# ElusAegis/metal-msm-gpu-acceleration

Hardware: AMD Instinct MI355X
Metric: BN254 G1 MSM/s at log_size=20 (5 instances) (higher is better)
Workload: dtype u32x8 (256-bit Montgomery integer)

## Files before the change

metal-msm-gpu-acceleration_amd/csrc/bn254_fq29.hip.h:

```cpp
#pragma once
#include "bn254_fq.hip.h"

namespace msm_amd {

struct fe29 {
  uint32_t l[9];
};

MSM_HD uint32_t limb32(uint32_t x) {
#if defined(__HIP_DEVICE_COMPILE__) && !defined(MSM_FQ29_NOPIN)
  asm("" : "+v"(x));
#endif
  return x;
}
MSM_HD fe29 pin_limbs(const fe29& a) {
  fe29 r;
#if defined(__HIP_DEVICE_COMPILE__)
  _Pragma("unroll") for (int i = 0; i < 9; ++i) r.l[i] = limb32(a.l[i]);
#else
  r = a;
#endif
  return r;
}

#if defined(__HIP_DEVICE_COMPILE__)
#define MSM_ISA_MARK(name) asm volatile("; MSM_MARK " name)
#else
#define MSM_ISA_MARK(name) ((void)0)
#endif

enum KSel { K4E30 = 0, K8E30 = 1, K8E31 = 2, K16E30 = 3, K16E31 = 4, K12E30 = 5 };

struct Fq29 {
  static constexpr uint32_t MASK = 0x1FFFFFFFu;
  static constexpr uint32_t INV = 0x04866389u;
  static constexpr uint32_t PINV = 0x1B799C77u;

  MSM_HD static constexpr uint32_t p(int i) {
    constexpr uint32_t c[9] = {0x187CFD47u, 0x010460B6u, 0x1C72A34Fu, 0x02D522D0u, 0x1585D978u,
                               0x02DB40C0u, 0x00A6E141u, 0x0E5C2634u, 0x0030644Eu};
    return c[i];
  }
  MSM_HD static constexpr uint32_t one_c(int i) {
    constexpr uint32_t c[9] = {0x157CCC21u, 0x141C2758u, 0x185230D3u, 0x014C0419u, 0x0AA36FB9u,
                               0x1D4240CEu, 0x11D54C07u, 0x052AC7A8u, 0x000DC836u};
    return c[i];
  }
  MSM_HD static constexpr uint32_t cin_c(int i) {
    constexpr uint32_t c[9] = {0x13349CA1u, 0x1A5D84A8u, 0x0A3E5CACu, 0x100249E0u, 0x12B951E8u,
                               0x0E92D304u, 0x14CB95B3u, 0x041B9D3Du, 0x00058003u};
    return c[i];
  }
  MSM_HD static constexpr uint32_t dout_c(int i) {
    constexpr uint32_t c[9] = {0x058F0D9Du, 0x1AEA1C6Eu, 0x11C2CF74u, 0x11D651EBu, 0x1462C0A7u,
                               0x11B7BC3Cu, 0x1CBD99BAu, 0x183340FBu, 0x000E0A77u};
    return c[i];
  }
  MSM_HD static constexpr uint32_t kc(int sel, int i) {
    constexpr uint32_t c[6][9] = {
        {0x41F3F51Cu, 0x441182D9u, 0x51CA8D3Au, 0x4B548B41u, 0x561765DEu, 0x4B6D0300u, 0x429B8502u, 0x597098CEu, 0x00C19137u},
        {0x43E7EA38u, 0x482305B4u, 0x43951A76u, 0x56A91685u, 0x4C2ECBBEu, 0x56DA0603u, 0x45370A06u, 0x52E1319Eu, 0x01832271u},
        {0x83E7EA38u, 0x882305B2u, 0x83951A74u, 0x96A91683u, 0x8C2ECBBCu, 0x96DA0601u, 0x85370A04u, 0x92E1319Cu, 0x0183226Fu},
        {0x47CFD470u, 0x50460B6Au, 0x472A34EEu, 0x4D522D0Cu, 0x585D977Fu, 0x4DB40C08u, 0x4A6E140Fu, 0x45C2633Eu, 0x030644E5u},
        {0x87CFD470u, 0x90460B68u, 0x872A34ECu, 0x8D522D0Au, 0x985D977Du, 0x8DB40C06u, 0x8A6E140Du, 0x85C2633Cu, 0x030644E3u},
        {0x45DBDF54u, 0x4C34888Fu, 0x555FA7B2u, 0x41FDA1C8u, 0x4246319Fu, 0x42470906u, 0x47D28F0Bu, 0x4C51CA6Eu, 0x0244B3ABu}};
    return c[sel][i];
  }

  MSM_HD static fe29 zero() {
    fe29 r;
    MSM_UNROLL for (int i = 0; i < 9; ++i) r.l[i] = 0;
    return r;
  }
  MSM_HD static fe29 one() {
    fe29 r;
    MSM_UNROLL for (int i = 0; i < 9; ++i) r.l[i] = one_c(i);
    return r;
  }
  MSM_HD static bool is_zero_limbs(const fe29& a) {
    uint32_t o = 0;
    MSM_UNROLL for (int i = 0; i < 9; ++i) o |= a.l[i];
    return o == 0;
  }

  MSM_HD static fe29 add(const fe29& a, const fe29& b) {
    fe29 r;
    MSM_UNROLL for (int i = 0; i < 9; ++i) r.l[i] = a.l[i] + b.l[i];
    return r;
  }

  template <int SEL>
  MSM_HD static fe29 sub(const fe29& a, const fe29& b) {
    fe29 r;
    MSM_UNROLL for (int i = 0; i < 9; ++i) r.l[i] = (a.l[i] + kc(SEL, i)) - b.l[i];
    return r;
  }

  MSM_HD static fe29 neg(const fe29& a) { return norm(sub<K4E30>(zero(), a)); }
  MSM_HD static fe29 neg_wide(const fe29& a) { return sub<K4E30>(zero(), a); }

  MSM_HD static fe29 norm(const fe29& a) {
    fe29 r;
    r.l[0] = a.l[0] & MASK;
    MSM_UNROLL for (int i = 1; i < 8; ++i) r.l[i] = (a.l[i] & MASK) + (a.l[i - 1] >> 29);
    r.l[8] = a.l[8] + (a.l[7] >> 29);
    return r;
  }

  template <bool WIDE = false>
  MSM_HD static fe29 reduce_columns(uint64_t (&A)[17]) {
    uint64_t carry = 0;
    MSM_UNROLL for (int k = 0; k < 9; ++k) {
      A[k] += carry;
      const uint32_t m = (WIDE && k < 8) ? (uint32_t)A[k] * INV : ((uint32_t)A[k] * INV) & MASK;
      MSM_UNROLL for (int j = 0; j < 9; ++j) A[k + j] += (uint64_t)m * p(j);
      carry = A[k] >> 29;
    }
    fe29 r;
    MSM_UNROLL for (int k = 9; k < 17; ++k) {
      A[k] += carry;
      r.l[k - 9] = (uint32_t)A[k] & MASK;
      carry = A[k] >> 29;
    }
    r.l[8] = (uint32_t)carry;
    return r;
  }


#if defined(MSM_AMD_EXPERIMENTS)
#include "experiments/fq29_variants.inc"
#endif

  template <bool PIN = true, bool WIDE = false>
  MSM_HD static fe29 mul(const fe29& a_in, const fe29& b_in) {
    const fe29 a = PIN ? pin_limbs(a_in) : a_in, b = PIN ? pin_limbs(b_in) : b_in;
#if defined(MSM_AMD_EXPERIMENTS) && defined(MSM_FQ29_FIPS)
    {
      const fe29* const xs[1] = {&a};
      const fe29* const ys[1] = {&b};
      return fips<1>(xs, ys);
    }
#endif
    uint64_t A[17];
    MSM_UNROLL for (int k = 0; k < 17; ++k) {
      uint64_t s = 0;
      MSM_UNROLL for (int i = 0; i < 9; ++i) {
        const int j = k - i;
        if (j >= 0 && j < 9) s += (uint64_t)a.l[i] * b.l[j];
      }
      A[k] = s;
    }
    return reduce_columns<WIDE>(A);
  }

  template <bool PIN = true, bool WIDE = false>
  MSM_HD static fe29 mul2(const fe29& a_in, const fe29& b_in, const fe29& c_in, const fe29& d_in) {
    const fe29 a = PIN ? pin_limbs(a_in) : a_in, b = PIN ? pin_limbs(b_in) : b_in, c = PIN ? pin_limbs(c_in) : c_in,
               d = PIN ? pin_limbs(d_in) : d_in;
#if defined(MSM_AMD_EXPERIMENTS) && defined(MSM_FQ29_FIPS)
    {
      const fe29* const xs[2] = {&a, &c};
      const fe29* const ys[2] = {&b, &d};
      return fips<2>(xs, ys);
    }
#endif
    uint64_t A[17];
    MSM_UNROLL for (int k = 0; k < 17; ++k) {
      uint64_t s = 0;
      MSM_UNROLL for (int i = 0; i < 9; ++i) {
        const int j = k - i;
        if (j >= 0 && j < 9) {
          s += (uint64_t)a.l[i] * b.l[j];
          s += (uint64_t)c.l[i] * d.l[j];
        }
      }
      A[k] = s;
    }
    return reduce_columns<WIDE>(A);
  }

  template <bool PIN = true, bool WIDE = false>
  MSM_HD static fe29 sqr(const fe29& a_in) {
    const fe29 a = PIN ? pin_limbs(a_in) : a_in;
#if defined(MSM_AMD_EXPERIMENTS) && defined(MSM_FQ29_FIPS)
    {
      fe29 d2;
      MSM_UNROLL for (int i = 0; i < 9; ++i) d2.l[i] = a.l[i] << 1;
      const fe29* const xs[1] = {&d2};
      const fe29* const ys[1] = {&a};
      return fips<1, true>(xs, ys);
    }
#endif
    uint32_t d[9];
    MSM_UNROLL for (int i = 0; i < 9; ++i) d[i] = a.l[i] << 1;
    uint64_t A[17];
    MSM_UNROLL for (int k = 0; k < 17; ++k) {
      uint64_t s = 0;
      MSM_UNROLL for (int i = 0; i < 9; ++i) {
        const int j = k - i;
        if (j >= 0 && j < 9 && i < j) s += (uint64_t)d[i] * a.l[j];
      }
      if ((k & 1) == 0) s += (uint64_t)a.l[k >> 1] * a.l[k >> 1];
      A[k] = s;
    }
    return reduce_columns<WIDE>(A);
  }
  MSM_HD static fe29 mul_np(const fe29& a, const fe29& b) { return mul<false, true>(a, b); }
  MSM_HD static fe29 sqr_np(const fe29& a) { return sqr<false, true>(a); }
  MSM_HD static fe29 mul2_np(const fe29& a, const fe29& b, const fe29& c, const fe29& d) { return mul2<false>(a, b, c, d); }
  MSM_HD static fe29 mul2w_np(const fe29& a, const fe29& b, const fe29& c, const fe29& d) {
    return mul2<false, true>(a, b, c, d);
  }

  MSM_HD static fe29 unpack256(const u256& x) {
    fe29 t;
    MSM_UNROLL for (int i = 0; i < 9; ++i) {
      const int bit = 29 * i;
      const int w = bit >> 5, s = bit & 31;
      uint32_t v = x.v[w] >> s;
      if (s > 3 && w + 1 < 8) v |= x.v[w + 1] << (32 - s);
      t.l[i] = (i < 8) ? (v & MASK) : v;
    }
    return t;
  }

  template <int SH>
  MSM_HD static fe29 unpack256_shl(const u256& x) {
    static_assert(SH >= 0 && SH <= 3, "the top limb holds 232 - SH .. 255 of x");
    fe29 t;
    t.l[0] = (x.v[0] << SH) & MASK;
    MSM_UNROLL for (int i = 1; i < 9; ++i) {
      const int bit = 29 * i - SH;
      const int w = bit >> 5, s = bit & 31;
      uint32_t v = x.v[w] >> s;
      if (s > 3 && w + 1 < 8) v |= x.v[w + 1] << (32 - s);
      t.l[i] = (i < 8) ? (v & MASK) : v;
    }
    return t;
  }

  MSM_HD static u256 pack256(const fe29& t) {
    u256 r;
    MSM_UNROLL for (int w = 0; w < 8; ++w) {
      const int bit = 32 * w;
      const int i = bit / 29, s = bit % 29;
      uint32_t v = t.l[i] >> s;
      if (i + 1 < 9) v |= t.l[i + 1] << (29 - s);
      if (29 - s + 29 < 32 && i + 2 < 9) v |= t.l[i + 2] << (58 - s);
      r.v[w] = v;
    }
    return r;
  }

  MSM_HD static fe29 from_ext(const u256& x) {
    fe29 c;
    MSM_UNROLL for (int i = 0; i < 9; ++i) c.l[i] = cin_c(i);
    return mul(unpack256(x), c);
  }

  MSM_HD static fe29 canonical(const fe29& a, int rounds) {
    fe29 r;
    uint32_t carry = 0;
    MSM_UNROLL for (int i = 0; i < 8; ++i) {
      const uint64_t s = (uint64_t)a.l[i] + carry;
      r.l[i] = (uint32_t)s & MASK;
      carry = (uint32_t)(s >> 29);
    }
    r.l[8] = a.l[8] + carry;
    for (int it = 0; it < rounds; ++it) {
      fe29 d;
      int32_t borrow = 0;
      MSM_UNROLL for (int i = 0; i < 9; ++i) {
        const int32_t s = (int32_t)r.l[i] - (int32_t)p(i) + borrow;
        d.l[i] = (i < 8) ? ((uint32_t)s & MASK) : (uint32_t)s;
        borrow = (i < 8) ? (s >> 29) : 0;
        if (i == 8) borrow = (s < 0) ? -1 : 0;
      }
      if (borrow == 0) r = d;
    }
    return r;
  }

  MSM_HD static u256 to_ext(const fe29& a) {
    fe29 d;
    MSM_UNROLL for (int i = 0; i < 9; ++i) d.l[i] = dout_c(i);
    return pack256(canonical(mul(a, d), 1));
  }

  MSM_HD static u256 pack_canonical(const fe29& a) { return pack256(canonical(a, 1)); }

  MSM_HD static bool maybe_zero(const fe29& a, uint32_t bound) {
    return (((a.l[0] & MASK) * PINV) & MASK) < bound;
  }

  MSM_HD static bool is_zero_exact(const fe29& a) {
    const fe29 t = canonical(mul(a, one()), 1);
    return is_zero_limbs(t);
  }
};

}
```

metal-msm-gpu-acceleration_amd/csrc/k_accumulate.hip:

```cpp
#include "device_common.hip.h"
#include "launch.h"
#include "point_stages.hip.h"

namespace msm_amd {

struct PackedBases {
  using Rec = AffPacked;
  static constexpr bool kIso = false;
  static __device__ __forceinline__ bool is_identity(const Rec& r) { return affpacked_is_identity(r); }
  static __device__ __forceinline__ AffI unpack(const Rec& r) { return affi_unpack_finite(r); }
  static __device__ __forceinline__ fe29 neg_y(const fe29& y) { return Fq29::neg_wide(y); }
};
struct ExtBases {
  using Rec = Affine;
  static constexpr bool kIso = true;
  static __device__ __forceinline__ bool is_identity(const Rec& r) { return affine_words_zero(r); }
  static __device__ __forceinline__ AffI unpack(const Rec& r) { return affi_from_ext_iso(r); }
  static __device__ __forceinline__ fe29 neg_y(const fe29& y) { return neg_wide_iso(y); }
};
template <bool PIN, class B>
__device__ __forceinline__ void
accumulate_item(const uint32_t slot, const typename B::Rec* __restrict__ bases, const uint32_t* __restrict__ sorted,
                   const uint32_t* __restrict__ bucket_start, const uint32_t* __restrict__ bucket_size,
                   const uint32_t* __restrict__ item_start, const uint32_t* __restrict__ win_base,
                   const uint2* __restrict__ order, const PlanCounters* __restrict__ counters, uint32_t n,
                   uint32_t lb, uint32_t CH, PtI* __restrict__ buckets, PtI* __restrict__ partials) {
  if (PIN) asm volatile("v_mov_b32 v175, 0" ::: "v175");
  if (slot >= counters->total_items) return;
  const uint2 it = order[slot];
  const uint32_t b = it.x, j = it.y;
  const uint32_t w = b >> lb;
  const uint32_t size = bucket_size[b];
  const uint32_t lo = j * CH;
  const uint32_t cnt = min(size - lo, CH);
  const uint32_t* idx = sorted + (size_t)w * n + bucket_start[b] + lo;
  PtI acc = pti_identity();
  enum : uint32_t { kEmpty = 0, kOne = 1, kMany = 2 };
  uint32_t state = kEmpty;
  uint32_t cur_idx = idx[0];
  uint32_t next_idx = cnt > 1 ? idx[1] : 0u;
  using Rec = typename B::Rec;
  Rec pre;
  pre.x = load_u256(&bases[cur_idx & 0x7FFFFFFFu].x);
  pre.y = load_u256(&bases[cur_idx & 0x7FFFFFFFu].y);
  uint32_t i = 0;
  auto signed_point = [](const Rec& rec, uint32_t entry) {
    AffI r = B::unpack(rec);
    const bool negate = (entry >> 31) != 0;
    const fe29 ny = B::neg_y(r.y);
#pragma unroll
    for (int l = 0; l < 9; ++l) r.y.l[l] = negate ? ny.l[l] : r.y.l[l];
    return r;
  };
  auto regather = [&](uint32_t entry) {
    Rec rec;
    rec.x = load_u256(&bases[entry & 0x7FFFFFFFu].x);
    rec.y = load_u256(&bases[entry & 0x7FFFFFFFu].y);
    return signed_point(rec, entry);
  };
  auto take = [&](AffI& cur) -> bool {
    const bool ident = B::is_identity(pre);
    cur = signed_point(pre, cur_idx);
    asm volatile("" : "+v"(cur.x.l[0]), "+v"(cur.x.l[1]), "+v"(cur.x.l[2]), "+v"(cur.x.l[3]), "+v"(cur.x.l[4]),
                      "+v"(cur.x.l[5]), "+v"(cur.x.l[6]), "+v"(cur.x.l[7]), "+v"(cur.x.l[8]), "+v"(cur.y.l[0]),
                      "+v"(cur.y.l[1]), "+v"(cur.y.l[2]), "+v"(cur.y.l[3]), "+v"(cur.y.l[4]), "+v"(cur.y.l[5]),
                      "+v"(cur.y.l[6]), "+v"(cur.y.l[7]), "+v"(cur.y.l[8]) :: "memory");
    cur_idx = next_idx;
    if (i + 1 < cnt) {
      pre.x = load_u256(&bases[cur_idx & 0x7FFFFFFFu].x);
      pre.y = load_u256(&bases[cur_idx & 0x7FFFFFFFu].y);
    }
    if (i + 2 < cnt) next_idx = idx[i + 2];
    ++i;
    return ident;
  };
  while (i < cnt) {
#pragma unroll 1
    while (i < cnt && state != kMany) {
      AffI cur;
      const uint32_t this_idx = cur_idx;
      if (take(cur)) continue;
      if (state == kOne) {
        MSM_ISA_MARK("begin affine_start");
        bool vanished = false;
        fe29 P, R;
        pti_mmadd_head<B::kIso>(acc.x, acc.y, cur.x, cur.y, P, R);
        acc = pti_mmadd_tail<B::kIso>(acc.x, acc.y, P, R, [&]() { return regather(this_idx); }, vanished);
        state = vanished ? (uint32_t)kEmpty : (uint32_t)kMany;
        MSM_ISA_MARK("end");
      } else {
        acc = pti_from_affi(cur);
        state = kOne;
      }
    }
#pragma unroll 1
    while (i < cnt) {
      AffI cur;
      const uint32_t this_idx = cur_idx;
      if (take(cur)) continue;
      MSM_ISA_MARK("begin mixed_addition");
      bool vanished = false;
      fe29 U2, S2;
      pti_madd_head(acc, cur.x, cur.y, U2, S2);
      acc = pti_madd_tail(acc, U2, S2, [&]() { return regather(this_idx); }, vanished);
      MSM_ISA_MARK("end");
      if (vanished) {
        state = kEmpty;
        break;
      }
    }
  }
  if (size <= CH) {
    store_pti(&buckets[b], acc);
  } else {
    store_pti(&partials[(size_t)win_base[w] + item_start[b] + j], acc);
  }
}

#define MSM_ACC_PARAMS_OF(Rec) const Rec* __restrict__ bases, const uint32_t* __restrict__ sorted,                    \
                       const uint32_t* __restrict__ bucket_start, const uint32_t* __restrict__ bucket_size,           \
                       const uint32_t* __restrict__ item_start, const uint32_t* __restrict__ win_base,                \
                       const uint2* __restrict__ order, const PlanCounters* __restrict__ counters, uint32_t n,        \
                       uint32_t lb, uint32_t CH, PtI* __restrict__ buckets, PtI* __restrict__ partials
#define MSM_ACC_PARAMS MSM_ACC_PARAMS_OF(AffPacked)
#define MSM_ACC_FWD bases, sorted, bucket_start, bucket_size, item_start, win_base, order, counters, n, lb, CH, buckets, partials
template <bool PIN, class B>
__global__ void __launch_bounds__(64) accumulate_kernel(MSM_ACC_PARAMS_OF(typename B::Rec)) {
  accumulate_item<PIN, B>(blockIdx.x * blockDim.x + threadIdx.x, MSM_ACC_FWD);
}
#if defined(MSM_AMD_EXPERIMENTS)
#include "experiments/k_accumulate_variants.inc"
#endif

__global__ void __launch_bounds__(64)
combine_small_kernel(const uint32_t* __restrict__ multi_list, PlanCounters* __restrict__ counters,
                     const uint32_t* __restrict__ bucket_size, const uint32_t* __restrict__ item_start,
                     const uint32_t* __restrict__ win_base, uint32_t lb, uint32_t CH,
                     const PtI* __restrict__ partials, PtI* __restrict__ buckets, uint32_t* __restrict__ big_list) {
  combine_small_body<G1Stages>(multi_list, counters, bucket_size, item_start, win_base, lb, CH, partials, buckets,
                               big_list);
}

__global__ void __launch_bounds__(64)
combine_big_kernel(const uint32_t* __restrict__ big_list, const PlanCounters* __restrict__ counters,
                   const uint32_t* __restrict__ bucket_size, const uint32_t* __restrict__ item_start,
                   const uint32_t* __restrict__ win_base, uint32_t lb, uint32_t CH,
                   const PtI* __restrict__ partials, PtI* __restrict__ buckets) {
  __shared__ PtI sh[64];
  combine_big_body<G1Stages>(sh, big_list, counters, bucket_size, item_start, win_base, lb, CH, partials, buckets);
}

void launch_accumulate(hipStream_t st, const Plan& p, const void* bases_any, int wide, const SortBuffers& b, PtI* buckets,
                       PtI* partials, int variant, uint32_t lds_bytes, hipEvent_t before_kernel, hipEvent_t after_kernel) {
  if (before_kernel) (void)hipEventRecord(before_kernel, st);
  const dim3 grid((unsigned)((p.max_items + 63) / 64)), block(64);
  const AffPacked* bases = (const AffPacked*)bases_any;
#if defined(MSM_AMD_EXPERIMENTS)
  if (wide) {
    hipLaunchKernelGGL(accumulate_kernel_wide, grid, block, lds_bytes, st, (const AffWide*)bases_any,
                       (const uint32_t*)b.sorted, (const uint32_t*)b.bucket_start, (const uint32_t*)b.bucket_size,
                       (const uint32_t*)b.item_start, (const uint32_t*)b.win_items, (const uint2*)b.order,
                       (const PlanCounters*)b.counters, p.n, p.lb, p.CH, buckets, partials);
    if (after_kernel) (void)hipEventRecord(after_kernel, st);
    return;
  }
#else
  (void)wide;
#endif
#define MSM_ACC_ARGS bases, (const uint32_t*)b.sorted, (const uint32_t*)b.bucket_start, (const uint32_t*)b.bucket_size, \
                     (const uint32_t*)b.item_start, (const uint32_t*)b.win_items, (const uint2*)b.order,                \
                     (const PlanCounters*)b.counters, p.n, p.lb, p.CH, buckets, partials
#if defined(MSM_AMD_EXPERIMENTS)
  if (variant == 4) {
    uint32_t* redo_list = b.redo_list;
    uint32_t* redo_count = &b.counters->pad[1];
    hipLaunchKernelGGL(accumulate_kernel_asm, grid, block, 0, st, MSM_ACC_ARGS, redo_list, redo_count);
    hipLaunchKernelGGL(accumulate_redo_kernel, dim3(1024), block, 0, st, MSM_ACC_ARGS, (const uint32_t*)redo_list,
                       (const uint32_t*)redo_count);
  } else if (variant == 2) {
    hipLaunchKernelGGL(accumulate_kernel_lean, grid, block, lds_bytes, st, MSM_ACC_ARGS);
  } else if (variant == 3) {
    hipLaunchKernelGGL(accumulate_kernel_w3, grid, block, lds_bytes, st, MSM_ACC_ARGS);
  } else if (variant == 5) {
    hipLaunchKernelGGL(accumulate_kernel_park, grid, block, 0, st, MSM_ACC_ARGS);
  } else if (variant == 10) {
    hipLaunchKernelGGL(accumulate_whatif_gathers, grid, block, lds_bytes, st, MSM_ACC_ARGS);
  } else if (variant == 11) {
    hipLaunchKernelGGL(accumulate_whatif_math, grid, block, lds_bytes, st, MSM_ACC_ARGS);
  } else if (variant == 12) {
    hipLaunchKernelGGL(accumulate_whatif_math_w3, grid, block, lds_bytes, st, MSM_ACC_ARGS);
  } else if (variant == 7) {
    hipLaunchKernelGGL(accumulate_kernel_r4, grid, block, lds_bytes, st, MSM_ACC_ARGS);
  } else
#endif
  if (p.on_iso) {
    const Affine* ext = (const Affine*)bases_any;
#define MSM_ACC_ARGS_EXT ext, (const uint32_t*)b.sorted, (const uint32_t*)b.bucket_start, (const uint32_t*)b.bucket_size, \
                         (const uint32_t*)b.item_start, (const uint32_t*)b.win_items, (const uint2*)b.order,             \
                         (const PlanCounters*)b.counters, p.n, p.lb, p.CH, buckets, partials
    if (variant == 1) {
      hipLaunchKernelGGL((accumulate_kernel<true, ExtBases>), grid, block, lds_bytes, st, MSM_ACC_ARGS_EXT);
    } else {
      hipLaunchKernelGGL((accumulate_kernel<false, ExtBases>), grid, block, lds_bytes, st, MSM_ACC_ARGS_EXT);
    }
#undef MSM_ACC_ARGS_EXT
  } else if (variant == 1) {
    hipLaunchKernelGGL((accumulate_kernel<true, PackedBases>), grid, block, lds_bytes, st, MSM_ACC_ARGS);
  } else {
    hipLaunchKernelGGL((accumulate_kernel<false, PackedBases>), grid, block, lds_bytes, st, MSM_ACC_ARGS);
  }
#undef MSM_ACC_ARGS
  if (after_kernel) (void)hipEventRecord(after_kernel, st);
}

void launch_combine(hipStream_t st, const Plan& p, const SortBuffers& b, PtI* buckets, PtI* partials) {
  launch_combine_pair(st, p, b, buckets, partials, combine_small_kernel, combine_big_kernel);
}

}
```

Measured before the change: 846.2.

## Use friendly-digit Montgomery reduction in Fq29 and bound combine_big occupancy

Replaces the first seven Montgomery reduction steps in the 29-bit limb field multiply with a variant that multiplies each low digit by a precomputed constant (p' multiple) and folds it into the next column, removing the per-step m = A[k]*INV multiply and carry chain. It is on by default and can be switched back with a macro. It also adds a min-blocks hint of 3 to combine_big_kernel's launch bounds to steer register allocation. The change in reduction correctness depends on the constants and bounded column growth, and the occupancy hint may cause spills.

```diff
diff --git a/metal-msm-gpu-acceleration_amd/csrc/bn254_fq29.hip.h b/metal-msm-gpu-acceleration_amd/csrc/bn254_fq29.hip.h
--- a/metal-msm-gpu-acceleration_amd/csrc/bn254_fq29.hip.h
+++ b/metal-msm-gpu-acceleration_amd/csrc/bn254_fq29.hip.h
@@ -107,10 +107,40 @@
     return r;
   }
 
-  template <bool WIDE = false>
+  MSM_HD static constexpr uint32_t npp(int i) {
+    constexpr uint32_t c[9] = {0x0872952Du, 0x0808854Au, 0x065124E0u, 0x029B9885u, 0x03F6B850u,
+                               0x148E9764u, 0x02B3E954u, 0x0843F777u, 0x0067A061u};
+    return c[i];
+  }
+  static constexpr int FRIENDLY_DIGITS = 7;
+#if defined(MSM_FQ29_CLASSIC_REDC)
+  static constexpr bool FRIENDLY_DEFAULT = false;
+#else
+  static constexpr bool FRIENDLY_DEFAULT = true;
+#endif
+  MSM_HD static uint32_t carry_factor() {
+    uint32_t eight = 8;
+#if defined(__HIP_DEVICE_COMPILE__)
+    asm("" : "+s"(eight));
+#endif
+    return eight;
+  }
+  template <bool WIDE = false, bool FRIENDLY = FRIENDLY_DEFAULT>
   MSM_HD static fe29 reduce_columns(uint64_t (&A)[17]) {
     uint64_t carry = 0;
     MSM_UNROLL for (int k = 0; k < 9; ++k) {
+      if (FRIENDLY && k < FRIENDLY_DIGITS) {
+        if (WIDE) {
+          const uint32_t m = (uint32_t)A[k], hi = (uint32_t)(A[k] >> 32);
+          MSM_UNROLL for (int j = 0; j < 9; ++j) A[k + 1 + j] += (uint64_t)m * npp(j);
+          A[k + 1] += (uint64_t)hi * carry_factor();
+        } else {
+          const uint32_t m = (uint32_t)A[k] & MASK;
+          MSM_UNROLL for (int j = 0; j < 9; ++j) A[k + 1 + j] += (uint64_t)m * npp(j);
+          A[k + 1] += A[k] >> 29;
+        }
+        continue;
+      }
       A[k] += carry;
       const uint32_t m = (WIDE && k < 8) ? (uint32_t)A[k] * INV : ((uint32_t)A[k] * INV) & MASK;
       MSM_UNROLL for (int j = 0; j < 9; ++j) A[k + j] += (uint64_t)m * p(j);
@@ -125,7 +155,6 @@
     r.l[8] = (uint32_t)carry;
     return r;
   }
-
 
 #if defined(MSM_AMD_EXPERIMENTS)
 #include "experiments/fq29_variants.inc"
diff --git a/metal-msm-gpu-acceleration_amd/csrc/k_accumulate.hip b/metal-msm-gpu-acceleration_amd/csrc/k_accumulate.hip
--- a/metal-msm-gpu-acceleration_amd/csrc/k_accumulate.hip
+++ b/metal-msm-gpu-acceleration_amd/csrc/k_accumulate.hip
@@ -141,7 +141,7 @@
                                big_list);
 }
 
-__global__ void __launch_bounds__(64)
+__global__ void __launch_bounds__(64, 3)
 combine_big_kernel(const uint32_t* __restrict__ big_list, const PlanCounters* __restrict__ counters,
                    const uint32_t* __restrict__ bucket_size, const uint32_t* __restrict__ item_start,
                    const uint32_t* __restrict__ win_base, uint32_t lb, uint32_t CH,
```

Result: faster. 881.5, median of 6 (+4.2%).
